# atonderski/future-object-detection

Measured on AMD Instinct MI355X. Metric: frame-sequences/sec fwd+bwd, T=6 900x1600, higher is better.
Workload: dtype bf16; 1 GPU; spatiotemporal ConditionalDETR (ResNet-50, 6 enc + 6 dec layers, 128 queries), T=6 frames 900x1600, batch 2/GPU, num_images K=5 (5 past frames live), random-init weights; step = forward (incl. Hungarian set loss, post-proc, AP bookkeeping) + backward + clip + AdamW; global_batch=2, frames=6, num_images=5, parallelism=dp1

## Files before the change

### future-object-detection_amd/csrc/api.cpp

```cpp
#include <stdarg.h>
#include <stdio.h>
#include <stdlib.h>
#include <string.h>

#include <mutex>

#include "../../include/fod.h"
#include "knobs.h"

static thread_local char g_err[512] = "";

void fod_set_error(const char* fmt, ...) {
  va_list ap;
  va_start(ap, fmt);
  vsnprintf(g_err, sizeof(g_err), fmt, ap);
  va_end(ap);
}

extern "C" size_t fod_last_error(char* buf, size_t cap) {
  const size_t n = strlen(g_err);
  if (buf && cap) {
    const size_t c = n < cap - 1 ? n : cap - 1;
    memcpy(buf, g_err, c);
    buf[c] = 0;
  }
  return n;
}

extern "C" int fod_abi_version(void) { return FOD_ABI_VERSION; }

extern "C" size_t fod_workspace_bytes(int kind) {
  switch (kind) {
    case FOD_WS_NT_SPLIT: return (size_t)FOD_NT_SPLIT_WS_FLOATS * sizeof(float);
    case FOD_WS_NT_SPLIT_TICKETS: return (size_t)FOD_NT_SPLIT_TICKETS * sizeof(unsigned);
    case FOD_WS_TN_PARTIALS: return FOD_TN_WS_BYTES;
    case FOD_WS_ATTN_SPLIT_PER_TILE: return (size_t)FOD_ATTN_SPLIT_WS_FLOATS_PER_TILE * sizeof(float);
    case FOD_WS_DET: return FOD_DET_WS_BYTES;
    case FOD_WS_TN_MULTI_DET: return FOD_TN_MULTI_DET_WS_BYTES;
    default: return 0;
  }
}

namespace {
struct KnobName {
  const char* name;
  int Knobs::*i;
  double Knobs::*d;
};
const KnobName KNOB_NAMES[] = {
    {"FOD_NT_SMALL", &Knobs::nt_small, nullptr},
    {"FOD_NT_NARROW", &Knobs::nt_narrow, nullptr},
    {"FOD_NT_SPLITK", &Knobs::nt_splitk, nullptr},
    {"FOD_NT_BIG", &Knobs::nt_big, nullptr},
    {"FOD_NT_BIG256", &Knobs::nt_big256, nullptr},
    {"FOD_NT_BIG_ILV", &Knobs::nt_big_ilv, nullptr},
    {"FOD_NT_BIG256_MINK", &Knobs::nt_big256_mink, nullptr},
    {"FOD_NT_BIG_MINK", &Knobs::nt_big_mink, nullptr},
    {"FOD_NT_BIG_MINN", &Knobs::nt_big_minn, nullptr},
    {"FOD_TN_SMALL", &Knobs::tn_small, nullptr},
    {"FOD_TN_BIG", &Knobs::tn_big, nullptr},
    {"FOD_TN_BIG_DENSE", &Knobs::tn_big_dense, nullptr},
    {"FOD_TN_BIG256", &Knobs::tn_big256, nullptr},
    {"FOD_TN_BIG_MIN", nullptr, &Knobs::tn_big_min},
    {"FOD_TN_BIG_SPLITS", &Knobs::tn_big_splits, nullptr},
    {"FOD_TN_WS", &Knobs::tn_ws, nullptr},
    {"FOD_TN_XCD", &Knobs::tn_xcd, nullptr},
    {"FOD_TN_ROWS", &Knobs::tn_rows, nullptr},
    {"FOD_ATTN_LDS", &Knobs::attn_lds, nullptr},
    {"FOD_ATTN_PF", &Knobs::attn_pf, nullptr},
    {"FOD_FP8_STAGE", &Knobs::fp8_stage, nullptr},
    {"FOD_LN_BWD_GROUPS", &Knobs::ln_bwd_groups, nullptr},
    {"FOD_BNK_VERSION", &Knobs::bnk_version, nullptr},
};

bool knob_parse(const KnobName& k, const char* text, Knobs& t) {
  char* end = nullptr;
  if (k.d) {
    const double v = strtod(text, &end);
    if (end == text || *end) return false;
    t.*k.d = v;
    return true;
  }
  if (Knobs{}.*k.i == Knobs::AUTO && !strcmp(text, "auto")) {
    t.*k.i = Knobs::AUTO;
    return true;
  }
  const long v = strtol(text, &end, 10);
  if (end == text || *end || v < 0 || v > 0x7FFFFFFF) return false;
  t.*k.i = (int)v;
  return true;
}

std::mutex g_knob_mutex;
Knobs& knob_table() {
  static Knobs table = [] {
    Knobs t;
    for (const KnobName& k : KNOB_NAMES)
      if (const char* text = getenv(k.name)) knob_parse(k, text, t);
    return t;
  }();
  return table;
}
const KnobName* knob_find(const char* name) {
  for (const KnobName& k : KNOB_NAMES)
    if (name && !strcmp(name, k.name)) return &k;
  fod_set_error("knob: unknown name %s", name ? name : "(null)");
  return nullptr;
}
}

Knobs fod_knobs() {
// ... 37 lines not shown
```

### future-object-detection_amd/csrc/gemm_nt.h

```cpp
#pragma once
#include "common.h"
#include "knobs.h"

namespace fodnt {

enum { MODE_DENSE = 0, MODE_CONV = 1, MODE_DGRAD = 2, MODE_DGRAD_S2 = 3, MODE_STEM = 4 };

struct NtParams {
  const void* A;
  const void* B;
  void* C;
  long lda, ldb, ldc;
  int M, N, K;
  int a_row_mod;
  const float* scale;
  const float* shift;
  const void* res;
  long ldr;
  int res_row_mod;
  const void* mask;
  long ldmask;
  int relu;
  int c_is_f32;
  int vec_epi;
  unsigned a_bytes, b_bytes;
  int gx, gy;
  int a_seg_len, c_seg_cols;
  long a_seg_stride, c_seg_stride;
  int par_h, par_w, out_H, out_W;
  int r_first, s_first, n_s;
  int off_h, off_w;
  int ksplit;
  float* split_ws;
  unsigned* split_tickets;
  int batches;
  long a_batch, b_batch, c_batch, shift_batch, res_batch, mask_batch;
  int res_nseg;
  long res_seg_stride;
  int Hs, Ws, Cs;
  int Hd, Wd;
  int kh, kw, stride, pad;
};

constexpr int BM = 128;
constexpr int ROW_BYTES = 128;

FOD_DEVINL int lds_off(int row, int chunk) { return row * ROW_BYTES + ((chunk ^ ((row >> 1) & 7)) << 4); }

constexpr int BMB = 256, BKB_EL = 64;

typedef fod_nt_route NtRoute;
NtRoute route(int mode, int dtype, const NtParams& p, const Knobs& kn);
int launch_big(int mode, const NtParams& p, const NtRoute& r, hipStream_t stream);

}
```

### future-object-detection_amd/csrc/gemm_nt.hip

```cpp
#include <stdlib.h>

#include <type_traits>

#include "common.h"
#include "gemm_nt.h"
#include "gemm_tn.h"

namespace {

using namespace fodnt;

template <typename T, int MODE, int NT, bool UTAP>
FOD_DEVINL void gemm_nt_body(const NtParams& p) {
  constexpr int VEC = Elem<T>::VEC;
  constexpr int BK = ROW_BYTES / (int)sizeof(T);
  constexpr int BN = 64 * NT;
  constexpr int KSTEPS = BK / 16;
  constexpr int BROWS = BN / 32;
  extern __shared__ __attribute__((aligned(16))) unsigned char smem[];
  unsigned char* sA = smem;
  unsigned char* sB = smem + 2 * BM * ROW_BYTES;

  const int tid = threadIdx.x;
  const int lane = tid & 63;
// ... 203 lines not shown
#pragma unroll
    for (int j = 0; j < NT; ++j) {
      const int row = wn * (32 * NT) + j * 32 + fr;
      if (sizeof(T) == 2) {
        const uint4 v = *reinterpret_cast<const uint4*>(b_s + lds_off(row, 2 * ks + fh));
        __builtin_memcpy(&fb[j], &v, 16);
      } else {
        const uint4 v0 = *reinterpret_cast<const uint4*>(b_s + lds_off(row, 4 * ks + 2 * fh));
        const uint4 v1 = *reinterpret_cast<const uint4*>(b_s + lds_off(row, 4 * ks + 2 * fh + 1));
        __builtin_memcpy(reinterpret_cast<char*>(&fb[j]), &v0, 16);
        __builtin_memcpy(reinterpret_cast<char*>(&fb[j]) + 16, &v1, 16);
      }
    }
  };
  auto compute = [&](int buf) {
    Frag<T> fa[2][2], fb[2][NT];
    read_frags(buf, 0, fa[0], fb[0]);
#pragma unroll
    for (int ks = 0; ks < KSTEPS; ++ks) {
      if (ks + 1 < KSTEPS) read_frags(buf, ks + 1, fa[(ks + 1) & 1], fb[(ks + 1) & 1]);
#pragma unroll
      for (int i = 0; i < 2; ++i)
#pragma unroll
        for (int j = 0; j < NT; ++j) mma16(fa[ks & 1][i], fb[ks & 1][j], acc[i][j]);
    }
  };
#define FOD_NT_STEP(k, LD, ST)                        \
  if ((k) < nkt) {                                    \
    if ((k) + 2 < nkt) load_tile((k) + 2, LD);        \
    compute((k) & 1);                                 \
    if ((k) + 1 < nkt) store_tile(((k) + 1) & 1, ST); \
    __syncthreads();                                  \
  }
  for (int kt = 0; kt < nkt; kt += 3) {
    FOD_NT_STEP(kt, st2, st1)
    FOD_NT_STEP(kt + 1, st0, st2)
    FOD_NT_STEP(kt + 2, st1, st0)
  }
#undef FOD_NT_STEP
  FOD_STAMP(3);

  const T* __restrict__ Rp = reinterpret_cast<const T*>(p.res);
  const T* __restrict__ Mp = reinterpret_cast<const T*>(p.mask);
  auto out_row = [&](int m) -> long {
    if (MODE != MODE_DGRAD_S2) return m;
    const int hw = p.Hd * p.Wd;
    const int img = m / hw;
    const int rem = m - img * hw;
    const int hq = rem / p.Wd;
    const int wq = rem - hq * p.Wd;
    return ((long)img * p.out_H + 2 * hq + p.par_h) * p.out_W + 2 * wq + p.par_w;
  };
  if (p.vec_epi) {
    typedef typename std::conditional<sizeof(T) == 2, bf16x4_t, f32x4>::type VT;
    constexpr int CPR = BN / 4;
    constexpr int RPP = 256 / CPR;
    constexpr int NPASS = BM / RPP;
    constexpr int PB = sizeof(T) == 2 ? NPASS : NPASS / 2;
    const int cq = tid % CPR, rq = tid / CPR;
    const int n = n0 + cq * 4;
    const int nc = min(n, p.N - 4);
    VT rres[PB], rmsk[PB];
    auto prefetch = [&](int base) {
#pragma unroll
      for (int ps = 0; ps < PB; ++ps) {
        const long m = out_row(min(m0 + rq + (base + ps) * RPP, p.M - 1));
        if (Rp) {
          const long rm = p.res_row_mod > 0 ? (m % p.res_row_mod) : m;
          rres[ps] = *reinterpret_cast<const VT*>(Rp + rm * p.ldr + nc);
        }
        if (Mp) rmsk[ps] = *reinterpret_cast<const VT*>(Mp + m * p.ldmask + nc);
      }
    };
    prefetch(0);
    float* sC = reinterpret_cast<float*>(smem);
#pragma unroll
    for (int i = 0; i < 2; ++i)
#pragma unroll
      for (int j = 0; j < NT; ++j)
#pragma unroll
        for (int r = 0; r < 16; ++r)
          sC[(wm * 64 + i * 32 + acc_row(r, lane)) * BN + wn * (32 * NT) + j * 32 + fr] = acc[i][j][r];
    FOD_STAMP(5);
    __syncthreads();
    FOD_STAMP(6);
    f32x4 sc = {1.f, 1.f, 1.f, 1.f}, sh = {0.f, 0.f, 0.f, 0.f};
    if (p.scale) sc = *reinterpret_cast<const f32x4*>(p.scale + nc);
    if (p.shift) sh = *reinterpret_cast<const f32x4*>(p.shift + nc);
    if (sizeof(T) == 2 && !p.c_is_f32 && PB == NPASS && m0 + BM <= p.M && n0 + BN <= p.N) {
      auto rows_out = [&](auto has_res, auto do_relu, auto has_mask) {
        f32x4 v[NPASS];
#pragma unroll
        for (int ps = 0; ps < NPASS; ++ps) v[ps] = *reinterpret_cast<const f32x4*>(sC + (rq + ps * RPP) * BN + cq * 4);
#pragma unroll
        for (int ps = 0; ps < NPASS; ++ps) {
          f32x4 w = v[ps] * sc + sh;
#pragma unroll
          for (int e = 0; e < 4; ++e) {
            if constexpr (decltype(has_res)::value) w[e] += (float)rres[ps][e];
            if constexpr (decltype(do_relu)::value) w[e] = fmaxf(w[e], 0.f);
            if constexpr (decltype(has_mask)::value) w[e] = ((float)rmsk[ps][e] > 0.f) ? w[e] : 0.f;
          }
          const long mo = out_row(m0 + rq + ps * RPP);
          *reinterpret_cast<bf16x4_t*>(reinterpret_cast<__bf16*>(p.C) + mo * p.ldc + n) =
              bf16x4_t{(__bf16)w[0], (__bf16)w[1], (__bf16)w[2], (__bf16)w[3]};
        }
      };
      typedef std::true_type Y;
      typedef std::false_type N_;
      const bool R = Rp != nullptr, L = p.relu != 0, K = Mp != nullptr;
      bool done = true;
      if (!R && !L && !K) rows_out(N_{}, N_{}, N_{});
      else if (!R && L && !K) rows_out(N_{}, Y{}, N_{});
      else if (R && L && !K) rows_out(Y{}, Y{}, N_{});
      else if (R && !L && !K) rows_out(Y{}, N_{}, N_{});
      else if (!R && !L && K) rows_out(N_{}, N_{}, Y{});
      else if (R && !L && K) rows_out(Y{}, N_{}, Y{});
      else done = false;
      if (done) {
        FOD_STAMP(4);
        return;
      }
    }
#pragma unroll
    for (int base = 0; base < NPASS; base += PB) {
      if (base > 0) prefetch(base);
#pragma unroll
      for (int ps = 0; ps < PB; ++ps) {
        const int row = rq + (base + ps) * RPP;
        const int m = m0 + row;
        f32x4 v = *reinterpret_cast<const f32x4*>(sC + row * BN + cq * 4);
        v = v * sc + sh;
        if (Rp) {
#pragma unroll
          for (int e = 0; e < 4; ++e) v[e] += (float)rres[ps][e];
        }
        if (p.relu) {
#pragma unroll
          for (int e = 0; e < 4; ++e) v[e] = fmaxf(v[e], 0.f);
        }
        if (Mp) {
#pragma unroll
          for (int e = 0; e < 4; ++e) v[e] = ((float)rmsk[ps][e] > 0.f) ? v[e] : 0.f;
        }
        if (m < p.M && n < p.N) {
          const long mo = out_row(m);
          if (p.c_is_f32 || sizeof(T) == 4) {
            *reinterpret_cast<f32x4*>(reinterpret_cast<float*>(p.C) + mo * p.ldc + n) = v;
          } else {
            *reinterpret_cast<bf16x4_t*>(reinterpret_cast<__bf16*>(p.C) + mo * p.ldc + n) =
                bf16x4_t{(__bf16)v[0], (__bf16)v[1], (__bf16)v[2], (__bf16)v[3]};
          }
        }
      }
    }
    FOD_STAMP(4);
    return;
  }
#pragma unroll
  for (int j = 0; j < NT; ++j) {
    const int n = n0 + wn * (32 * NT) + j * 32 + fr;
    if (n >= p.N) continue;
    const float sc = p.scale ? p.scale[n] : 1.f;
    const float sh = p.shift ? p.shift[n] : 0.f;
#pragma unroll
    for (int i = 0; i < 2; ++i) {
#pragma unroll
      for (int r = 0; r < 16; ++r) {
        const int mt = m0 + wm * 64 + i * 32 + acc_row(r, lane);
        if (mt >= p.M) continue;
        const long m = out_row(mt);
        float v = acc[i][j][r] * sc + sh;
        if (Rp) {
          const long rm = p.res_row_mod > 0 ? (m % p.res_row_mod) : m;
          v += to_f32(Rp[rm * p.ldr + n]);
        }
        if (p.relu) v = fmaxf(v, 0.f);
        if (Mp) v = (to_f32(Mp[m * p.ldmask + n]) > 0.f) ? v : 0.f;
        if (p.c_is_f32)
          reinterpret_cast<float*>(p.C)[m * p.ldc + n] = v;
        else
          reinterpret_cast<T*>(p.C)[m * p.ldc + n] = from_f32<T>(v);
      }
    }
// ... 243 lines not shown
    if (narrow) hipLaunchKernelGGL((KERNEL_NT1), grid, block, lds, stream, q);       \
    else hipLaunchKernelGGL((KERNEL_NT2), grid, block, lds, stream, q);              \
  } while (0)
  if constexpr (MODE == MODE_DENSE) {
    FOD_NT_LAUNCH((gemm_nt_kernel<T, 1>), (gemm_nt_kernel<T, 2>));
  } else if constexpr (MODE == MODE_STEM) {
    FOD_NT_LAUNCH((conv_stem_fwd_kernel<T, 1>), (conv_stem_fwd_kernel<T, 2>));
  } else if constexpr (MODE == MODE_CONV) {
    if (utap) FOD_NT_LAUNCH((conv2d_fwd_kernel<T, 1, true>), (conv2d_fwd_kernel<T, 2, true>));
    else FOD_NT_LAUNCH((conv2d_fwd_kernel<T, 1, false>), (conv2d_fwd_kernel<T, 2, false>));
  } else if constexpr (MODE == MODE_DGRAD) {
    if (utap) FOD_NT_LAUNCH((conv2d_dgrad_kernel<T, 1, true>), (conv2d_dgrad_kernel<T, 2, true>));
    else FOD_NT_LAUNCH((conv2d_dgrad_kernel<T, 1, false>), (conv2d_dgrad_kernel<T, 2, false>));
  } else {
    if (utap) FOD_NT_LAUNCH((conv2d_dgrad_s2_kernel<T, 1, true>), (conv2d_dgrad_s2_kernel<T, 2, true>));
    else FOD_NT_LAUNCH((conv2d_dgrad_s2_kernel<T, 1, false>), (conv2d_dgrad_s2_kernel<T, 2, false>));
  }
#undef FOD_NT_LAUNCH
  FOD_LAUNCH_CHECK();
  return FOD_OK;
}

template <int MODE>
int launch(int dtype, const NtParams& p, hipStream_t stream) {
  if (dtype != FOD_BF16 && dtype != FOD_F32) {
    fod_set_error("gemm_nt: bad dtype %d", dtype);
    return FOD_ERR_ARG;
  }
  const NtRoute r = route(MODE, dtype, p, fod_knobs());
  if (r.kernel == FOD_ROUTE_NT_BIG) return launch_big(MODE, p, r, stream);
  if (r.kernel == FOD_ROUTE_NT_128)
    return dtype == FOD_BF16 ? launch_128<__bf16, MODE>(p, r, stream) : launch_128<float, MODE>(p, r, stream);
  NtParams q = p;
  q.ksplit = r.ksplit > 1 ? r.ksplit : 0;
  hipLaunchKernelGGL(gemm_nt_small_kernel, dim3(ceil_div(p.N, 64), ceil_div(p.M, 64), r.ksplit), dim3(256), 0, stream, q);
  FOD_LAUNCH_CHECK();
  return FOD_OK;
}

void fill_epilogue(NtParams& p, const fod_epilogue* e) {
  p.scale = e ? e->scale : nullptr;
  p.shift = e ? e->shift : nullptr;
  p.res = e ? e->residual : nullptr;
  p.ldr = e ? e->ld_residual : 0;
  p.res_row_mod = e ? e->residual_row_mod : 0;
  p.mask = e ? e->relu_mask : nullptr;
  p.ldmask = e ? e->ld_mask : 0;
  p.relu = e ? e->relu : 0;
  p.c_is_f32 = e ? e->out_f32 : 0;
  p.split_ws = e ? reinterpret_cast<float*>(e->split_ws) : nullptr;
  p.split_tickets = e ? reinterpret_cast<unsigned*>(e->split_tickets) : nullptr;
}

void decide_vec_epilogue(NtParams& p) {
  auto al = [](const void* q) { return ((uintptr_t)q % 16) == 0; };
  p.vec_epi = (p.N % 4 == 0) && (p.ldc % 4 == 0) && al(p.C) && (!p.scale || al(p.scale)) &&
              (!p.shift || al(p.shift)) && (!p.res || (p.ldr % 4 == 0 && al(p.res))) &&
              (!p.mask || (p.ldmask % 4 == 0 && al(p.mask)));
}

}

namespace fodnt {
namespace {
bool small_applies(int dtype, const NtParams& p, const Knobs& kn) {
  if (!kn.nt_small) return false;
  if (dtype != FOD_BF16 || !p.vec_epi) return false;
  const long blocks = (long)ceil_div(p.M, 64) * ceil_div(p.N, 64);
  if (blocks > 256) return false;
  if (p.res && ((long)(p.res_row_mod > 0 ? p.res_row_mod : p.M) * p.ldr + p.N) * 2 >= 0x7FFFFFF0L) return false;
  if (p.mask && ((long)p.M * p.ldmask + p.N) * 2 >= 0x7FFFFFF0L) return false;
  return true;
}

bool big256_applies(const NtParams& p, const Knobs& kn) {
  if (kn.nt_big256 == 0) return false;
  if (p.N < 256) return false;
  if (kn.nt_big256 == 2) return true;
  const long tiles = (long)ceil_div(p.M, BMB) * ceil_div(p.N, 256);
  return p.N % 256 == 0 && tiles >= 200;
}

bool big_applies(int mode, const NtParams& p, const Knobs& kn) {
  if (kn.nt_big == 0) return false;
  if (!p.vec_epi || p.a_seg_len || p.c_seg_cols) return false;
  if (mode == MODE_STEM) return false;
  if (mode != MODE_DENSE && (p.Cs % BKB_EL != 0 || p.K < BKB_EL)) return false;
  if (mode == MODE_DENSE && p.K % 8 != 0) return false;
  if (p.N % 4 != 0) return false;
  const long tiles = (long)ceil_div(p.M, BMB) * ceil_div(p.N, 128);
  if (kn.nt_big == 2) return true;
  if (mode != MODE_DENSE && p.K >= kn.nt_big256_mink && p.K < 1536 && big256_applies(p, kn)) return true;
  return p.K >= kn.nt_big_mink && p.N >= kn.nt_big_minn && tiles >= 200;
}
}

NtRoute route(int mode, int dtype, const NtParams& p, const Knobs& kn) {
  NtRoute r{};
  r.ksplit = 1;
  if (mode == MODE_DENSE && small_applies(dtype, p, kn)) {
    r.kernel = FOD_ROUTE_NT_SMALL;
    r.tile_n = 64;
    const long tiles = (long)ceil_div(p.N, 64) * ceil_div(p.M, 64);
    if (p.K >= 1024 && tiles <= 64 && kn.nt_splitk != 0) {
      const int cap = kn.nt_splitk > 1 ? (kn.nt_splitk < 8 ? kn.nt_splitk : 8) : 4;
      int ks = (int)(256 / tiles);
      if (ks > cap) ks = cap;
      if (ks > p.K / 256) ks = p.K / 256;
      r.wants_split_ws = ks > 1;
      if (ks > 1 && p.split_ws && p.split_tickets) r.ksplit = ks;
    }
// ... 155 lines not shown
  const int Wo = (g->W + 2 * g->pad - g->kw) / g->stride + 1;
  FOD_REQUIRE(Ho == g->Ho && Wo == g->Wo, "conv: geometry mismatch Ho=%d/%d Wo=%d/%d", g->Ho, Ho, g->Wo, Wo);
  FOD_REQUIRE(g->Cin % vec == 0 && g->Cout % vec == 0, "conv: channels %d/%d must be multiples of %d",
              g->Cin, g->Cout, vec);
  FOD_REQUIRE(((uintptr_t)src % 16) == 0 && ((uintptr_t)w % 16) == 0, "conv: operands must be 16-byte aligned");
  p.A = src; p.B = w; p.C = dst;
  p.kh = g->kh; p.kw = g->kw; p.stride = g->stride; p.pad = g->pad;
  if (!dgrad) {
    p.Hs = g->H; p.Ws = g->W; p.Cs = g->Cin;
    p.Hd = g->Ho; p.Wd = g->Wo;
    p.M = g->Nimg * g->Ho * g->Wo;
    p.N = g->Cout;
    p.K = g->kh * g->kw * g->Cin;
  } else {
    p.Hs = g->Ho; p.Ws = g->Wo; p.Cs = g->Cout;
    p.Hd = g->H; p.Wd = g->W;
    p.M = g->Nimg * g->H * g->W;
    p.N = g->Cin;
    p.K = g->kh * g->kw * g->Cout;
  }
  FOD_REQUIRE((long)g->Nimg * g->H * g->W < (1L << 31) && (long)g->Nimg * g->Ho * g->Wo < (1L << 31),
              "conv: pixel count overflows int");
  p.ldb = p.K;
  p.ldc = p.N;
  fill_epilogue(p, epi);
  decide_vec_epilogue(p);
  const long esz = dtype == FOD_BF16 ? 2 : 4;
  const long ab = (long)g->Nimg * p.Hs * p.Ws * p.Cs * esz, bb = (long)p.N * p.K * esz;
  FOD_REQUIRE(ab < 0xFFFFFFF0L - 16 && bb < 0xFFFFFFF0L - 16, "conv: operand larger than 4 GiB");
  p.a_bytes = (unsigned)ab;
  p.b_bytes = (unsigned)bb;
  return FOD_OK;
}

bool dgrad_s2_class(NtParams& q, const NtParams& p, const fod_conv_geom* g, int cls) {
  q = p;
  q.out_H = g->H;
  q.out_W = g->W;
  q.par_h = cls >> 1;
  q.par_w = cls & 1;
  q.Hd = (g->H - q.par_h + 1) / 2;
  q.Wd = (g->W - q.par_w + 1) / 2;
  if (q.Hd <= 0 || q.Wd <= 0) return false;
  q.r_first = (q.par_h + g->pad) & 1;
  q.s_first = (q.par_w + g->pad) & 1;
  const int n_r = q.r_first < g->kh ? (g->kh - q.r_first + 1) / 2 : 0;
  q.n_s = q.s_first < g->kw ? (g->kw - q.s_first + 1) / 2 : 0;
  q.off_h = (q.par_h + g->pad - q.r_first) / 2;
  q.off_w = (q.par_w + g->pad - q.s_first) / 2;
  q.M = g->Nimg * q.Hd * q.Wd;
  q.K = n_r * q.n_s * g->Cout;
  if (q.K == 0 && p.res == p.C && p.res != nullptr && !p.scale && !p.shift && !p.relu && p.ldr == p.ldc) return false;
  if (q.n_s == 0) q.n_s = 1;
  return true;
}

int conv_common(int dtype, bool dgrad, const void* src, const void* w, void* dst, const fod_conv_geom* g,
                const fod_epilogue* epi, hipStream_t stream) {
  FOD_REQUIRE(src && w && dst && g, "conv: null operand");
  NtParams p{};
  if (int rc = conv_params(p, dtype, dgrad, src, w, dst, g, epi)) return rc;
  if (!dgrad) return launch<MODE_CONV>(dtype, p, stream);
  if (g->stride == 1) return launch<MODE_DGRAD>(dtype, p, stream);
  for (int cls = 0; cls < 4; ++cls) {
    NtParams q;
    if (!dgrad_s2_class(q, p, g, cls)) continue;
    if (int rc = launch<MODE_DGRAD_S2>(dtype, q, stream)) return rc;
  }
  return FOD_OK;
}

int conv_route(int dtype, bool dgrad, const fod_conv_geom* g, const fod_epilogue* epi, fod_nt_route* out) {
  FOD_REQUIRE(out && g && (dtype == FOD_BF16 || dtype == FOD_F32), "conv2d_route: bad args");
  NtParams p{};
  if (int rc = conv_params(p, dtype, dgrad, nullptr, nullptr, nullptr, g, epi)) return rc;
  int mode = dgrad ? MODE_DGRAD : MODE_CONV;
  if (dgrad && g->stride == 2) {
    NtParams q;
    FOD_REQUIRE(dgrad_s2_class(q, p, g, 0), "conv2d_route: parity class (0, 0) has no launch");
    p = q;
    mode = MODE_DGRAD_S2;
  }
  *out = route(mode, dtype, p, fod_knobs());
  return FOD_OK;
}
}

extern "C" int fod_conv2d_route(int which, int dtype, const fod_conv_geom* g, const fod_epilogue* epi, int det,
                                size_t ws_bytes, void* out) {
  if (which == FOD_CONV_WGRAD) return fodtn::conv_wgrad_route(dtype, g, det, ws_bytes, reinterpret_cast<fod_tn_route*>(out));
  FOD_REQUIRE(which == FOD_CONV_FWD || which == FOD_CONV_DGRAD, "conv2d_route: which = %d", which);
  return conv_route(dtype, which == FOD_CONV_DGRAD, g, epi, reinterpret_cast<fod_nt_route*>(out));
}

extern "C" int fod_conv2d_fwd(int dtype, const void* x, const void* w, void* y, const fod_conv_geom* g,
                              const fod_epilogue* epi, hipStream_t stream) {
  return conv_common(dtype, false, x, w, y, g, epi, stream);
}

extern "C" int fod_conv2d_dgrad(int dtype, const void* dy, const void* w_t, void* dx, const fod_conv_geom* g,
                                const fod_epilogue* epi, hipStream_t stream) {
  return conv_common(dtype, true, dy, w_t, dx, g, epi, stream);
}

extern "C" int fod_conv_stem_fwd(int dtype, const void* xp, const void* w, void* y, int Nimg, int Hp, int Wp, int Ho,
                                 int Wo, int Cout, const fod_epilogue* epi, hipStream_t stream) {
// ... 28 lines not shown
```

### future-object-detection_amd/csrc/gemm_nt_big.hip

```cpp
#include <type_traits>

#include "common.h"
#include "gemm_nt.h"
#include "lds_dma.h"

namespace {

using namespace fodnt;

constexpr int A_DMA = BMB / 64;
template <int MODE, int BNB, int NSTAGE, bool ILV>
__global__ __launch_bounds__(512) void nt_big_kernel(const NtParams p) {
  constexpr int STAGE_BYTES = (BMB + BNB) * ROW_BYTES;
  constexpr int B_DMA = BNB / 64;
  constexpr int N_DMA = A_DMA + B_DMA;
  constexpr int NJ = BNB / 64;
  static_assert((BNB == 128 && NSTAGE == 3) || (BNB == 256 && NSTAGE == 2), "tile shapes: 256 x 128 x 3 stages, 256 x 256 x 2");
  typedef __bf16 T;
  constexpr unsigned ESZ = 2;
  constexpr unsigned BKB = BKB_EL * ESZ;
  constexpr int KSTEPS = BKB_EL / 16;
  extern __shared__ __attribute__((aligned(16))) unsigned char smem[];

  const int tid = threadIdx.x;
// ... 188 lines not shown
        if constexpr (ILV) {
          __builtin_amdgcn_sched_barrier(0);
          issue_idx(fill, 2 * ks + i);
          __builtin_amdgcn_sched_barrier(0);
        }
      }
    }
  };

  auto wait_landed = [&](auto with_lgkm) {
    if constexpr (NSTAGE == 3) {
      static_assert(N_DMA == 6, "vmcnt immediate");
      if constexpr (decltype(with_lgkm)::value) asm volatile("s_waitcnt vmcnt(6) lgkmcnt(0)" ::: "memory");
      else asm volatile("s_waitcnt vmcnt(6)" ::: "memory");
    } else {
      if constexpr (decltype(with_lgkm)::value) asm volatile("s_waitcnt vmcnt(0) lgkmcnt(0)" ::: "memory");
      else asm volatile("s_waitcnt vmcnt(0)" ::: "memory");
    }
  };
  const int nkt = (p.K + BKB_EL - 1) / BKB_EL;
#pragma unroll
  for (int t = 0; t < NSTAGE - 1; ++t) issue_tile(t);
  wait_landed(std::false_type{});
  __builtin_amdgcn_s_barrier();
  int st_c = 0, st_i = NSTAGE - 1;
  for (int kt = 0; kt < nkt; ++kt) {
    const TileCtx fill = begin_tile(st_i);
    if constexpr (!ILV) {
#pragma unroll
      for (int idx = 0; idx < N_DMA; ++idx) issue_idx(fill, idx);
    }
    compute(st_c, fill);
    wait_landed(std::true_type{});
    __builtin_amdgcn_s_barrier();
    st_c = st_c == NSTAGE - 1 ? 0 : st_c + 1;
    st_i = st_i == NSTAGE - 1 ? 0 : st_i + 1;
  }
  asm volatile("s_waitcnt vmcnt(0)" ::: "memory");
  __builtin_amdgcn_s_barrier();

  const T* __restrict__ Rp = reinterpret_cast<const T*>(p.res);
  const T* __restrict__ Mp = reinterpret_cast<const T*>(p.mask);
  auto out_row = [&](int m) -> long {
    if (MODE != MODE_DGRAD_S2) return m;
    const int hw = p.Hd * p.Wd;
    const int img = m / hw;
    const int rem = m - img * hw;
    const int hq = rem / p.Wd;
    const int wq = rem - hq * p.Wd;
    return ((long)img * p.out_H + 2 * hq + p.par_h) * p.out_W + 2 * wq + p.par_w;
  };
  constexpr int HALVES = (BMB * BNB * 4 > NSTAGE * STAGE_BYTES) ? 2 : 1;
  constexpr int ROWS_H = BMB / HALVES;
  constexpr int CPR = BNB / 4;
  constexpr int RPP = 512 / CPR;
  constexpr int NPASS = ROWS_H / RPP;
  constexpr int PB = 8;
  const int cq = tid % CPR, rq = tid / CPR;
  const int n = n0 + cq * 4;
  const int nc = min(n, p.N - 4);
  float* sC = reinterpret_cast<float*>(smem);
  f32x4 sc = {1.f, 1.f, 1.f, 1.f}, sh = {0.f, 0.f, 0.f, 0.f};
  if (p.scale) sc = *reinterpret_cast<const f32x4*>(p.scale + nc);
  if (p.shift) sh = *reinterpret_cast<const f32x4*>(p.shift + nc);
  const bool full = m0 + BMB <= p.M && n0 + BNB <= p.N && !p.c_is_f32;
  int mh = 0;
  auto rows_out = [&](auto has_res, auto do_relu, auto has_mask, auto is_full) {
#pragma unroll
    for (int base = 0; base < NPASS; base += PB) {
      bf16x4_t rres[PB], rmsk[PB];
      f32x4 v[PB];
#pragma unroll
      for (int ps = 0; ps < PB; ++ps) {
        const long m = out_row(min(m0 + mh + rq + (base + ps) * RPP, p.M - 1));
        if constexpr (decltype(has_res)::value) {
          const long rm = p.res_row_mod > 0 ? (m % p.res_row_mod) : m;
          rres[ps] = *reinterpret_cast<const bf16x4_t*>(Rp + rm * p.ldr + nc);
        }
        if constexpr (decltype(has_mask)::value) rmsk[ps] = *reinterpret_cast<const bf16x4_t*>(Mp + m * p.ldmask + nc);
      }
#pragma unroll
      for (int ps = 0; ps < PB; ++ps)
        v[ps] = *reinterpret_cast<const f32x4*>(sC + (rq + (base + ps) * RPP) * BNB + cq * 4);
#pragma unroll
      for (int ps = 0; ps < PB; ++ps) {
        f32x4 w = v[ps] * sc + sh;
#pragma unroll
        for (int e = 0; e < 4; ++e) {
          if constexpr (decltype(has_res)::value) w[e] += (float)rres[ps][e];
          if constexpr (decltype(do_relu)::value) w[e] = fmaxf(w[e], 0.f);
          if constexpr (decltype(has_mask)::value) w[e] = ((float)rmsk[ps][e] > 0.f) ? w[e] : 0.f;
        }
        const int mt = m0 + mh + rq + (base + ps) * RPP;
        if constexpr (!decltype(is_full)::value) {
          if (mt >= p.M || n >= p.N) continue;
        }
        const long mo = out_row(mt);
        if (decltype(is_full)::value || !p.c_is_f32) {
          *reinterpret_cast<bf16x4_t*>(reinterpret_cast<__bf16*>(p.C) + mo * p.ldc + n) =
              bf16x4_t{(__bf16)w[0], (__bf16)w[1], (__bf16)w[2], (__bf16)w[3]};
        } else {
          *reinterpret_cast<f32x4*>(reinterpret_cast<float*>(p.C) + mo * p.ldc + n) = w;
        }
      }
    }
  };
  typedef std::true_type Y;
  typedef std::false_type N_;
  const bool R = Rp != nullptr, L = p.relu != 0, K = Mp != nullptr;
  auto pick = [&](auto is_full) {
    if (!R && !L && !K) rows_out(N_{}, N_{}, N_{}, is_full);
    else if (!R && L && !K) rows_out(N_{}, Y{}, N_{}, is_full);
    else if (R && L && !K) rows_out(Y{}, Y{}, N_{}, is_full);
    else if (R && !L && !K) rows_out(Y{}, N_{}, N_{}, is_full);
    else if (!R && !L && K) rows_out(N_{}, N_{}, Y{}, is_full);
    else if (R && !L && K) rows_out(Y{}, N_{}, Y{}, is_full);
    else if (!R && L && K) rows_out(N_{}, Y{}, Y{}, is_full);
    else rows_out(Y{}, Y{}, Y{}, is_full);
  };
#pragma unroll
  for (int h = 0; h < HALVES; ++h) {
    mh = h * ROWS_H;
    if (h > 0) __syncthreads();
    if (wm / (4 / HALVES) == h) {
#pragma unroll
      for (int i = 0; i < 2; ++i)
#pragma unroll
        for (int j = 0; j < NJ; ++j)
#pragma unroll
          for (int r = 0; r < 16; ++r)
            sC[((wm % (4 / HALVES)) * 64 + i * 32 + acc_row(r, lane)) * BNB + wn * (BNB / 2) + j * 32 + fr] = acc[i][j][r];
    }
    __syncthreads();
    if (full) pick(Y{});
    else pick(N_{});
  }
}

template <int MODE, int BNB, int NSTAGE, bool ILV>
int launch_big_ilv(const NtParams& q, hipStream_t stream) {
  static LdsLimitOnce lds_once;
  const size_t lds = (size_t)NSTAGE * (BMB + BNB) * ROW_BYTES;
  if (int rc = fod_lds_limit_once(lds_once, reinterpret_cast<const void*>(&nt_big_kernel<MODE, BNB, NSTAGE, ILV>), lds, "gemm_nt_big")) return rc;
  const dim3 grid(q.gx * ((q.gy + 7) / 8 * 8));
  hipLaunchKernelGGL((nt_big_kernel<MODE, BNB, NSTAGE, ILV>), grid, dim3(512), lds, stream, q);
  FOD_LAUNCH_CHECK();
  return FOD_OK;
}

template <int MODE>
int launch_big_mode(const NtParams& p, const NtRoute& r, hipStream_t stream) {
  NtParams q = p;
  q.gy = ceil_div(p.M, BMB);
  q.gx = ceil_div(p.N, r.tile_n);
  if (r.tile_n == 256)
    return r.interleave ? launch_big_ilv<MODE, 256, 2, true>(q, stream) : launch_big_ilv<MODE, 256, 2, false>(q, stream);
  return r.interleave ? launch_big_ilv<MODE, 128, 3, true>(q, stream) : launch_big_ilv<MODE, 128, 3, false>(q, stream);
}

}

namespace fodnt {

int launch_big(int mode, const NtParams& p, const NtRoute& r, hipStream_t stream) {
  switch (mode) {
    case MODE_DENSE: return launch_big_mode<MODE_DENSE>(p, r, stream);
    case MODE_CONV: return launch_big_mode<MODE_CONV>(p, r, stream);
    case MODE_DGRAD: return launch_big_mode<MODE_DGRAD>(p, r, stream);
    case MODE_DGRAD_S2: return launch_big_mode<MODE_DGRAD_S2>(p, r, stream);
    default: break;
  }
  fod_set_error("gemm_nt_big: unsupported mode %d", mode);
  return FOD_ERR_ARG;
}

}
```

### future-object-detection_amd/csrc/knobs.h

```cpp
#pragma once

struct Knobs {
  static constexpr int AUTO = -1;
  int nt_small = 1;
  int nt_narrow = AUTO;
  int nt_splitk = AUTO;
  int nt_big = 1;
  int nt_big256 = 1;
  int nt_big_ilv = AUTO;
  int nt_big256_mink = 128;
  int nt_big_mink = 1536;
  int nt_big_minn = 256;
  int tn_small = 1;
  int tn_big = 1;
  int tn_big_dense = 0;
  int tn_big256 = 0;
  double tn_big_min = 2.0e9;
  int tn_big_splits = 0;
  int tn_ws = 1;
  int tn_xcd = 1;
  int tn_rows = 0;
  int attn_lds = 8;
  int attn_pf = 1;
  int fp8_stage = 1;
  int ln_bwd_groups = 4;
  int bnk_version = 4;
};

Knobs fod_knobs();
```

Measured before the change: 109.6 frame-sequences/s.

## Add swizzled LDS staging and 16-byte fast-path GEMM epilogue with 32-bit offsets

Reworks the NT GEMM epilogues (small and big kernels). Accumulators are now staged into LDS with an XOR swizzle to cut bank conflicts. Full tiles take a new fast path that uses 32-bit byte offsets, preloads residual and mask, and writes 8-wide bf16 vectors (16-byte stores) when alignment permits. The fast path also covers stride-2 dgrad row remapping through incremental offset advancing. This adds code size, register pressure and a new knob, and relies on an overflow check for the 32-bit offsets.

```diff
diff --git a/future-object-detection_amd/csrc/api.cpp b/future-object-detection_amd/csrc/api.cpp
--- a/future-object-detection_amd/csrc/api.cpp
+++ b/future-object-detection_amd/csrc/api.cpp
@@ -57,6 +57,7 @@
     {"FOD_NT_BIG256_MINK", &Knobs::nt_big256_mink, nullptr},
     {"FOD_NT_BIG_MINK", &Knobs::nt_big_mink, nullptr},
     {"FOD_NT_BIG_MINN", &Knobs::nt_big_minn, nullptr},
+    {"FOD_NT_EPI16", &Knobs::nt_epi16, nullptr},
     {"FOD_TN_SMALL", &Knobs::tn_small, nullptr},
     {"FOD_TN_BIG", &Knobs::tn_big, nullptr},
     {"FOD_TN_BIG_DENSE", &Knobs::tn_big_dense, nullptr},
diff --git a/future-object-detection_amd/csrc/gemm_nt.h b/future-object-detection_amd/csrc/gemm_nt.h
--- a/future-object-detection_amd/csrc/gemm_nt.h
+++ b/future-object-detection_amd/csrc/gemm_nt.h
@@ -23,6 +23,8 @@
   int relu;
   int c_is_f32;
   int vec_epi;
+  int epi_off32;
+  int epi16;
   unsigned a_bytes, b_bytes;
   int gx, gy;
   int a_seg_len, c_seg_cols;
@@ -47,6 +49,10 @@
 
 FOD_DEVINL int lds_off(int row, int chunk) { return row * ROW_BYTES + ((chunk ^ ((row >> 1) & 7)) << 4); }
 
+FOD_DEVINL int stage_idx(int idx) { return idx ^ ((idx >> 5) & 4); }
+template <int BN>
+FOD_DEVINL int stage_flip(int r, int wn) { return (BN == 64 ? (r >> 1) & 1 : BN == 128 ? r & 1 : wn) << 2; }
+
 constexpr int BMB = 256, BKB_EL = 64;
 
 typedef fod_nt_route NtRoute;
diff --git a/future-object-detection_amd/csrc/gemm_nt.hip b/future-object-detection_amd/csrc/gemm_nt.hip
--- a/future-object-detection_amd/csrc/gemm_nt.hip
+++ b/future-object-detection_amd/csrc/gemm_nt.hip
@@ -279,6 +279,131 @@
     return ((long)img * p.out_H + 2 * hq + p.par_h) * p.out_W + 2 * wq + p.par_w;
   };
   if (p.vec_epi) {
+    float* sC = reinterpret_cast<float*>(smem);
+    auto stage_acc = [&]() __attribute__((always_inline)) {
+#pragma unroll
+      for (int i = 0; i < 2; ++i)
+#pragma unroll
+        for (int j = 0; j < NT; ++j)
+#pragma unroll
+          for (int r = 0; r < 16; ++r)
+            sC[(wm * 64 + i * 32 + acc_row(r, lane)) * BN + wn * (32 * NT) + j * 32 + (fr ^ stage_flip<BN>(r, wn))] =
+                acc[i][j][r];
+    };
+    if constexpr (sizeof(T) == 2) {
+      const bool R = Rp != nullptr, L = p.relu != 0, K = Mp != nullptr;
+      if (p.epi_off32 && !p.c_is_f32 && !(L && K) && p.res_row_mod == 0 && m0 + BM <= p.M && n0 + BN <= p.N) {
+        auto fast_tile = [&](auto w_) __attribute__((always_inline)) {
+          constexpr int W = decltype(w_)::value;
+          typedef typename std::conditional<W == 8, bf16x8_t, bf16x4_t>::type VB;
+          constexpr int CPR = BN / W;
+          constexpr int RPP = 256 / CPR;
+          constexpr int NPASS = BM / RPP;
+          const int cq = tid % CPR, rq = tid / CPR;
+          const unsigned ldcB = (unsigned)p.ldc * 2u, ldrB = (unsigned)p.ldr * 2u, ldmB = (unsigned)p.ldmask * 2u;
+          long row0 = m0;
+          int hq = 0, wq = 0;
+          unsigned d = (unsigned)rq;
+          const unsigned d_row = (unsigned)(2 * p.out_W - 2 * p.Wd);
+          const unsigned d_img = (unsigned)((p.out_H - 2 * p.Hd) * p.out_W);
+          auto advance = [&](int rows) __attribute__((always_inline)) {
+            wq += rows;
+            d += 2u * (unsigned)rows;
+            while (wq >= p.Wd) {
+              wq -= p.Wd;
+              d += d_row;
+              if (++hq == p.Hd) {
+                hq = 0;
+                d += d_img;
+              }
+            }
+          };
+          if (MODE == MODE_DGRAD_S2) {
+            const int hw = p.Hd * p.Wd;
+            const int img = m0 / hw;
+            const int rem = m0 - img * hw;
+            hq = rem / p.Wd;
+            wq = rem - hq * p.Wd;
+            row0 = ((long)img * p.out_H + 2 * hq + p.par_h) * p.out_W + 2 * wq + p.par_w;
+            d = 0;
+            advance(rq);
+          }
+          char* Cb = reinterpret_cast<char*>(p.C) + (row0 * p.ldc + n0) * 2;
+          const char* Rb = reinterpret_cast<const char*>(Rp) + (row0 * p.ldr + n0) * 2;
+          const char* Mb = reinterpret_cast<const char*>(Mp) + (row0 * p.ldmask + n0) * 2;
+          const unsigned col = (unsigned)(cq * W) * 2u;
+          unsigned offC[NPASS], oc = 0, orr = 0, om = 0;
+          VB rres[NPASS], rmsk[NPASS];
+#pragma unroll
+          for (int ps = 0; ps < NPASS; ++ps) {
+            if (MODE == MODE_DGRAD_S2 || ps == 0) {
+              oc = d * ldcB + col;
+              orr = d * ldrB + col;
+              om = d * ldmB + col;
+            }
+            offC[ps] = oc;
+            if (Rp) rres[ps] = *reinterpret_cast<const VB*>(Rb + orr);
+            if (Mp) rmsk[ps] = *reinterpret_cast<const VB*>(Mb + om);
+            if (MODE == MODE_DGRAD_S2) {
+              if (ps + 1 < NPASS) advance(RPP);
+            } else {
+              oc += RPP * ldcB;
+              orr += RPP * ldrB;
+              om += RPP * ldmB;
+            }
+          }
+          stage_acc();
+          FOD_STAMP(5);
+          __syncthreads();
+          FOD_STAMP(6);
+          f32x4 sc[W / 4], sh[W / 4];
+#pragma unroll
+          for (int h = 0; h < W / 4; ++h) {
+            sc[h] = f32x4{1.f, 1.f, 1.f, 1.f};
+            sh[h] = f32x4{0.f, 0.f, 0.f, 0.f};
+            if (p.scale) sc[h] = *reinterpret_cast<const f32x4*>(p.scale + n0 + cq * W + 4 * h);
+            if (p.shift) sh[h] = *reinterpret_cast<const f32x4*>(p.shift + n0 + cq * W + 4 * h);
+          }
+          const int s0 = stage_idx(rq * BN + cq * W);
+          auto rows_out = [&](auto has_res, auto do_relu, auto has_mask) {
+            f32x4 v[NPASS][W / 4];
+#pragma unroll
+            for (int ps = 0; ps < NPASS; ++ps)
+#pragma unroll
+              for (int h = 0; h < W / 4; ++h)
+                v[ps][h] = *reinterpret_cast<const f32x4*>(sC + ps * RPP * BN + (s0 ^ (4 * h)));
+#pragma unroll
+            for (int ps = 0; ps < NPASS; ++ps) {
+              VB o;
+#pragma unroll
+              for (int h = 0; h < W / 4; ++h) {
+                f32x4 w = v[ps][h] * sc[h] + sh[h];
+#pragma unroll
+                for (int e = 0; e < 4; ++e) {
+                  if constexpr (decltype(has_res)::value) w[e] += (float)rres[ps][4 * h + e];
+                  if constexpr (decltype(do_relu)::value) w[e] = fmaxf(w[e], 0.f);
+                  if constexpr (decltype(has_mask)::value) w[e] = ((float)rmsk[ps][4 * h + e] > 0.f) ? w[e] : 0.f;
+                  o[4 * h + e] = (__bf16)w[e];
+                }
+              }
+              *reinterpret_cast<VB*>(Cb + offC[ps]) = o;
+            }
+          };
+          typedef std::true_type Y;
+          typedef std::false_type N_;
+          if (!R && !L && !K) rows_out(N_{}, N_{}, N_{});
+          else if (!R && L && !K) rows_out(N_{}, Y{}, N_{});
+          else if (R && L && !K) rows_out(Y{}, Y{}, N_{});
+          else if (R && !L && !K) rows_out(Y{}, N_{}, N_{});
+          else if (!R && !L && K) rows_out(N_{}, N_{}, Y{});
+          else rows_out(Y{}, N_{}, Y{});
+        };
+        if (MODE != MODE_STEM && p.epi16) fast_tile(std::integral_constant<int, 8>{});
+        else fast_tile(std::integral_constant<int, 4>{});
+        FOD_STAMP(4);
+        return;
+      }
+    }
     typedef typename std::conditional<sizeof(T) == 2, bf16x4_t, f32x4>::type VT;
     constexpr int CPR = BN / 4;
     constexpr int RPP = 256 / CPR;
@@ -300,55 +425,14 @@
       }
     };
     prefetch(0);
-    float* sC = reinterpret_cast<float*>(smem);
-#pragma unroll
-    for (int i = 0; i < 2; ++i)
-#pragma unroll
-      for (int j = 0; j < NT; ++j)
-#pragma unroll
-        for (int r = 0; r < 16; ++r)
-          sC[(wm * 64 + i * 32 + acc_row(r, lane)) * BN + wn * (32 * NT) + j * 32 + fr] = acc[i][j][r];
+    stage_acc();
     FOD_STAMP(5);
     __syncthreads();
     FOD_STAMP(6);
     f32x4 sc = {1.f, 1.f, 1.f, 1.f}, sh = {0.f, 0.f, 0.f, 0.f};
     if (p.scale) sc = *reinterpret_cast<const f32x4*>(p.scale + nc);
     if (p.shift) sh = *reinterpret_cast<const f32x4*>(p.shift + nc);
-    if (sizeof(T) == 2 && !p.c_is_f32 && PB == NPASS && m0 + BM <= p.M && n0 + BN <= p.N) {
-      auto rows_out = [&](auto has_res, auto do_relu, auto has_mask) {
-        f32x4 v[NPASS];
-#pragma unroll
-        for (int ps = 0; ps < NPASS; ++ps) v[ps] = *reinterpret_cast<const f32x4*>(sC + (rq + ps * RPP) * BN + cq * 4);
-#pragma unroll
-        for (int ps = 0; ps < NPASS; ++ps) {
-          f32x4 w = v[ps] * sc + sh;
-#pragma unroll
-          for (int e = 0; e < 4; ++e) {
-            if constexpr (decltype(has_res)::value) w[e] += (float)rres[ps][e];
-            if constexpr (decltype(do_relu)::value) w[e] = fmaxf(w[e], 0.f);
-            if constexpr (decltype(has_mask)::value) w[e] = ((float)rmsk[ps][e] > 0.f) ? w[e] : 0.f;
-          }
-          const long mo = out_row(m0 + rq + ps * RPP);
-          *reinterpret_cast<bf16x4_t*>(reinterpret_cast<__bf16*>(p.C) + mo * p.ldc + n) =
-              bf16x4_t{(__bf16)w[0], (__bf16)w[1], (__bf16)w[2], (__bf16)w[3]};
-        }
-      };
-      typedef std::true_type Y;
-      typedef std::false_type N_;
-      const bool R = Rp != nullptr, L = p.relu != 0, K = Mp != nullptr;
-      bool done = true;
-      if (!R && !L && !K) rows_out(N_{}, N_{}, N_{});
-      else if (!R && L && !K) rows_out(N_{}, Y{}, N_{});
-      else if (R && L && !K) rows_out(Y{}, Y{}, N_{});
-      else if (R && !L && !K) rows_out(Y{}, N_{}, N_{});
-      else if (!R && !L && K) rows_out(N_{}, N_{}, Y{});
-      else if (R && !L && K) rows_out(Y{}, N_{}, Y{});
-      else done = false;
-      if (done) {
-        FOD_STAMP(4);
-        return;
-      }
-    }
+    const int s0 = stage_idx(rq * BN + cq * 4);
 #pragma unroll
     for (int base = 0; base < NPASS; base += PB) {
       if (base > 0) prefetch(base);
@@ -356,7 +440,7 @@
       for (int ps = 0; ps < PB; ++ps) {
         const int row = rq + (base + ps) * RPP;
         const int m = m0 + row;
-        f32x4 v = *reinterpret_cast<const f32x4*>(sC + row * BN + cq * 4);
+        f32x4 v = *reinterpret_cast<const f32x4*>(sC + (base + ps) * RPP * BN + s0);
         v = v * sc + sh;
         if (Rp) {
 #pragma unroll
@@ -706,11 +790,23 @@
   p.split_tickets = e ? reinterpret_cast<unsigned*>(e->split_tickets) : nullptr;
 }
 
+void epilogue_span(NtParams& p, long rows);
+
 void decide_vec_epilogue(NtParams& p) {
   auto al = [](const void* q) { return ((uintptr_t)q % 16) == 0; };
   p.vec_epi = (p.N % 4 == 0) && (p.ldc % 4 == 0) && al(p.C) && (!p.scale || al(p.scale)) &&
               (!p.shift || al(p.shift)) && (!p.res || (p.ldr % 4 == 0 && al(p.res))) &&
               (!p.mask || (p.ldmask % 4 == 0 && al(p.mask)));
+  p.epi16 = p.vec_epi && fod_knobs().nt_epi16 != 0 && (p.N % 8 == 0) && (p.ldc % 8 == 0) && (!p.res || p.ldr % 8 == 0) &&
+            (!p.mask || p.ldmask % 8 == 0);
+  epilogue_span(p, BMB);
+}
+
+void epilogue_span(NtParams& p, long rows) {
+  long ld = p.ldc;
+  if (p.res && p.ldr > ld) ld = p.ldr;
+  if (p.mask && p.ldmask > ld) ld = p.ldmask;
+  p.epi_off32 = p.ldc >= 0 && p.ldr >= 0 && p.ldmask >= 0 && (rows + 1) * ld * 4 < 0xFFFFFFF0L;
 }
 
 }
@@ -972,6 +1068,7 @@
   q.K = n_r * q.n_s * g->Cout;
   if (q.K == 0 && p.res == p.C && p.res != nullptr && !p.scale && !p.shift && !p.relu && p.ldr == p.ldc) return false;
   if (q.n_s == 0) q.n_s = 1;
+  epilogue_span(q, 32L * BMB + 16L * q.out_W);
   return true;
 }
 
diff --git a/future-object-detection_amd/csrc/gemm_nt_big.hip b/future-object-detection_amd/csrc/gemm_nt_big.hip
--- a/future-object-detection_amd/csrc/gemm_nt_big.hip
+++ b/future-object-detection_amd/csrc/gemm_nt_big.hip
@@ -264,6 +264,138 @@
   };
   constexpr int HALVES = (BMB * BNB * 4 > NSTAGE * STAGE_BYTES) ? 2 : 1;
   constexpr int ROWS_H = BMB / HALVES;
+  float* sC = reinterpret_cast<float*>(smem);
+  auto stage_half = [&](int h) __attribute__((always_inline)) {
+    if (wm / (4 / HALVES) == h) {
+#pragma unroll
+      for (int i = 0; i < 2; ++i)
+#pragma unroll
+        for (int j = 0; j < NJ; ++j)
+#pragma unroll
+          for (int r = 0; r < 16; ++r)
+            sC[((wm % (4 / HALVES)) * 64 + i * 32 + acc_row(r, lane)) * BNB + wn * (BNB / 2) + j * 32 +
+               (fr ^ stage_flip<BNB>(r, wn))] = acc[i][j][r];
+    }
+  };
+  typedef std::true_type Y;
+  typedef std::false_type N_;
+  const bool R = Rp != nullptr, L = p.relu != 0, K = Mp != nullptr;
+  if (p.epi_off32 && !p.c_is_f32 && p.res_row_mod == 0 && m0 + BMB <= p.M && n0 + BNB <= p.N) {
+    auto fast_tile = [&](auto w_) __attribute__((always_inline)) {
+      constexpr int W = decltype(w_)::value;
+      typedef typename std::conditional<W == 8, bf16x8_t, bf16x4_t>::type VB;
+      constexpr int CPR = BNB / W;
+      constexpr int RPP = 512 / CPR;
+      constexpr int NPASS = ROWS_H / RPP;
+      constexpr int PB = 32 / W;
+      const int cq = tid % CPR, rq = tid / CPR;
+      const unsigned ldcB = (unsigned)p.ldc * 2u, ldrB = (unsigned)p.ldr * 2u, ldmB = (unsigned)p.ldmask * 2u;
+      long row0 = m0;
+      int hq = 0, wq = 0;
+      unsigned d = (unsigned)rq;
+      const unsigned d_row = (unsigned)(2 * p.out_W - 2 * p.Wd);
+      const unsigned d_img = (unsigned)((p.out_H - 2 * p.Hd) * p.out_W);
+      auto advance = [&](int rows) __attribute__((always_inline)) {
+        wq += rows;
+        d += 2u * (unsigned)rows;
+        while (wq >= p.Wd) {
+          wq -= p.Wd;
+          d += d_row;
+          if (++hq == p.Hd) {
+            hq = 0;
+            d += d_img;
+          }
+        }
+      };
+      if (MODE == MODE_DGRAD_S2) {
+        const int hw = p.Hd * p.Wd;
+        const int img = m0 / hw;
+        const int rem = m0 - img * hw;
+        hq = rem / p.Wd;
+        wq = rem - hq * p.Wd;
+        row0 = ((long)img * p.out_H + 2 * hq + p.par_h) * p.out_W + 2 * wq + p.par_w;
+        d = 0;
+        advance(rq);
+      }
+      char* Cb = reinterpret_cast<char*>(p.C) + (row0 * p.ldc + n0) * 2;
+      const char* Rb = reinterpret_cast<const char*>(Rp) + (row0 * p.ldr + n0) * 2;
+      const char* Mb = reinterpret_cast<const char*>(Mp) + (row0 * p.ldmask + n0) * 2;
+      const unsigned col = (unsigned)(cq * W) * 2u;
+      unsigned oc = d * ldcB + col, orr = d * ldrB + col, om = d * ldmB + col;
+      f32x4 sc[W / 4], sh[W / 4];
+#pragma unroll
+      for (int h = 0; h < W / 4; ++h) {
+        sc[h] = f32x4{1.f, 1.f, 1.f, 1.f};
+        sh[h] = f32x4{0.f, 0.f, 0.f, 0.f};
+        if (p.scale) sc[h] = *reinterpret_cast<const f32x4*>(p.scale + n0 + cq * W + 4 * h);
+        if (p.shift) sh[h] = *reinterpret_cast<const f32x4*>(p.shift + n0 + cq * W + 4 * h);
+      }
+      const int s0 = stage_idx(rq * BNB + cq * W);
+      auto rows_out = [&](auto has_res, auto do_relu, auto has_mask) {
+#pragma unroll
+        for (int base = 0; base < NPASS; base += PB) {
+          VB rres[PB], rmsk[PB];
+          unsigned offC[PB];
+          f32x4 v[PB][W / 4];
+#pragma unroll
+          for (int ps = 0; ps < PB; ++ps) {
+            offC[ps] = oc;
+            if constexpr (decltype(has_res)::value) rres[ps] = *reinterpret_cast<const VB*>(Rb + orr);
+            if constexpr (decltype(has_mask)::value) rmsk[ps] = *reinterpret_cast<const VB*>(Mb + om);
+            if (MODE == MODE_DGRAD_S2) {
+              advance(RPP);
+              oc = d * ldcB + col;
+              orr = d * ldrB + col;
+              om = d * ldmB + col;
+            } else {
+              oc += RPP * ldcB;
+              orr += RPP * ldrB;
+              om += RPP * ldmB;
+            }
+          }
+#pragma unroll
+          for (int ps = 0; ps < PB; ++ps)
+#pragma unroll
+            for (int h = 0; h < W / 4; ++h)
+              v[ps][h] = *reinterpret_cast<const f32x4*>(sC + (base + ps) * RPP * BNB + (s0 ^ (4 * h)));
+#pragma unroll
+          for (int ps = 0; ps < PB; ++ps) {
+            VB o;
+#pragma unroll
+            for (int h = 0; h < W / 4; ++h) {
+              f32x4 w = v[ps][h] * sc[h] + sh[h];
+#pragma unroll
+              for (int e = 0; e < 4; ++e) {
+                if constexpr (decltype(has_res)::value) w[e] += (float)rres[ps][4 * h + e];
+                if constexpr (decltype(do_relu)::value) w[e] = fmaxf(w[e], 0.f);
+                if constexpr (decltype(has_mask)::value) w[e] = ((float)rmsk[ps][4 * h + e] > 0.f) ? w[e] : 0.f;
+                o[4 * h + e] = (__bf16)w[e];
+              }
+            }
+            *reinterpret_cast<VB*>(Cb + offC[ps]) = o;
+          }
+        }
+      };
+      auto half_out = [&](int h) __attribute__((always_inline)) {
+        if (h > 0) __syncthreads();
+        stage_half(h);
+        __syncthreads();
+        if (!R && !L && !K) rows_out(N_{}, N_{}, N_{});
+        else if (!R && L && !K) rows_out(N_{}, Y{}, N_{});
+        else if (R && L && !K) rows_out(Y{}, Y{}, N_{});
+        else if (R && !L && !K) rows_out(Y{}, N_{}, N_{});
+        else if (!R && !L && K) rows_out(N_{}, N_{}, Y{});
+        else if (R && !L && K) rows_out(Y{}, N_{}, Y{});
+        else if (!R && L && K) rows_out(N_{}, Y{}, Y{});
+        else rows_out(Y{}, Y{}, Y{});
+      };
+      half_out(0);
+      if constexpr (HALVES == 2) half_out(1);
+    };
+    if (p.epi16) fast_tile(std::integral_constant<int, 8>{});
+    else fast_tile(std::integral_constant<int, 4>{});
+    return;
+  }
   constexpr int CPR = BNB / 4;
   constexpr int RPP = 512 / CPR;
   constexpr int NPASS = ROWS_H / RPP;
@@ -271,13 +403,12 @@
   const int cq = tid % CPR, rq = tid / CPR;
   const int n = n0 + cq * 4;
   const int nc = min(n, p.N - 4);
-  float* sC = reinterpret_cast<float*>(smem);
   f32x4 sc = {1.f, 1.f, 1.f, 1.f}, sh = {0.f, 0.f, 0.f, 0.f};
   if (p.scale) sc = *reinterpret_cast<const f32x4*>(p.scale + nc);
   if (p.shift) sh = *reinterpret_cast<const f32x4*>(p.shift + nc);
-  const bool full = m0 + BMB <= p.M && n0 + BNB <= p.N && !p.c_is_f32;
+  const int s0 = stage_idx(rq * BNB + cq * 4);
   int mh = 0;
-  auto rows_out = [&](auto has_res, auto do_relu, auto has_mask, auto is_full) {
+  auto rows_out = [&](auto has_res, auto do_relu, auto has_mask) {
 #pragma unroll
     for (int base = 0; base < NPASS; base += PB) {
       bf16x4_t rres[PB], rmsk[PB];
@@ -293,7 +424,7 @@
       }
 #pragma unroll
       for (int ps = 0; ps < PB; ++ps)
-        v[ps] = *reinterpret_cast<const f32x4*>(sC + (rq + (base + ps) * RPP) * BNB + cq * 4);
+        v[ps] = *reinterpret_cast<const f32x4*>(sC + (base + ps) * RPP * BNB + s0);
 #pragma unroll
       for (int ps = 0; ps < PB; ++ps) {
         f32x4 w = v[ps] * sc + sh;
@@ -304,11 +435,9 @@
           if constexpr (decltype(has_mask)::value) w[e] = ((float)rmsk[ps][e] > 0.f) ? w[e] : 0.f;
         }
         const int mt = m0 + mh + rq + (base + ps) * RPP;
-        if constexpr (!decltype(is_full)::value) {
-          if (mt >= p.M || n >= p.N) continue;
-        }
+        if (mt >= p.M || n >= p.N) continue;
         const long mo = out_row(mt);
-        if (decltype(is_full)::value || !p.c_is_f32) {
+        if (!p.c_is_f32) {
           *reinterpret_cast<bf16x4_t*>(reinterpret_cast<__bf16*>(p.C) + mo * p.ldc + n) =
               bf16x4_t{(__bf16)w[0], (__bf16)w[1], (__bf16)w[2], (__bf16)w[3]};
         } else {
@@ -317,36 +446,22 @@
       }
     }
   };
-  typedef std::true_type Y;
-  typedef std::false_type N_;
-  const bool R = Rp != nullptr, L = p.relu != 0, K = Mp != nullptr;
-  auto pick = [&](auto is_full) {
-    if (!R && !L && !K) rows_out(N_{}, N_{}, N_{}, is_full);
-    else if (!R && L && !K) rows_out(N_{}, Y{}, N_{}, is_full);
-    else if (R && L && !K) rows_out(Y{}, Y{}, N_{}, is_full);
-    else if (R && !L && !K) rows_out(Y{}, N_{}, N_{}, is_full);
-    else if (!R && !L && K) rows_out(N_{}, N_{}, Y{}, is_full);
-    else if (R && !L && K) rows_out(Y{}, N_{}, Y{}, is_full);
-    else if (!R && L && K) rows_out(N_{}, Y{}, Y{}, is_full);
-    else rows_out(Y{}, Y{}, Y{}, is_full);
-  };
-#pragma unroll
-  for (int h = 0; h < HALVES; ++h) {
+  auto half_out = [&](int h) __attribute__((always_inline)) {
     mh = h * ROWS_H;
     if (h > 0) __syncthreads();
-    if (wm / (4 / HALVES) == h) {
-#pragma unroll
-      for (int i = 0; i < 2; ++i)
-#pragma unroll
-        for (int j = 0; j < NJ; ++j)
-#pragma unroll
-          for (int r = 0; r < 16; ++r)
-            sC[((wm % (4 / HALVES)) * 64 + i * 32 + acc_row(r, lane)) * BNB + wn * (BNB / 2) + j * 32 + fr] = acc[i][j][r];
-    }
+    stage_half(h);
     __syncthreads();
-    if (full) pick(Y{});
-    else pick(N_{});
-  }
+    if (!R && !L && !K) rows_out(N_{}, N_{}, N_{});
+    else if (!R && L && !K) rows_out(N_{}, Y{}, N_{});
+    else if (R && L && !K) rows_out(Y{}, Y{}, N_{});
+    else if (R && !L && !K) rows_out(Y{}, N_{}, N_{});
+    else if (!R && !L && K) rows_out(N_{}, N_{}, Y{});
+    else if (R && !L && K) rows_out(Y{}, N_{}, Y{});
+    else if (!R && L && K) rows_out(N_{}, Y{}, Y{});
+    else rows_out(Y{}, Y{}, Y{});
+  };
+  half_out(0);
+  if constexpr (HALVES == 2) half_out(1);
 }
 
 template <int MODE, int BNB, int NSTAGE, bool ILV>
diff --git a/future-object-detection_amd/csrc/knobs.h b/future-object-detection_amd/csrc/knobs.h
--- a/future-object-detection_amd/csrc/knobs.h
+++ b/future-object-detection_amd/csrc/knobs.h
@@ -11,6 +11,7 @@
   int nt_big256_mink = 128;
   int nt_big_mink = 1536;
   int nt_big_minn = 256;
+  int nt_epi16 = 1;
   int tn_small = 1;
   int tn_big = 1;
   int tn_big_dense = 0;
```

Result: no change. 109.6 frame-sequences/s (median of 2 runs) (+0.0%).
